# VISION-SJTU/UniDefense

Measured on AMD Instinct MI355X. Metric: images/sec fwd+bwd (256x256, EffNet-b4), higher is better.
Workload: dtype f32

## Files before the change

unidefense_amd/csrc/conv_mfma.hip:

```cpp
#include "pw_common.h"

namespace {

typedef _Float16 f16x2 __attribute__((ext_vector_type(2)));
typedef _Float16 f16x8 __attribute__((ext_vector_type(8)));
typedef uint32_t u32x2 __attribute__((ext_vector_type(2)));


constexpr int odd_slots(int bytes) { return (bytes / 16) % 2 == 0 ? bytes + 16 : bytes; }
constexpr int round_up(int v, int m) { return (v + m - 1) / m * m; }

template <int CIN_, int COUT_, int MODE_, int TH_, int TW_, int CK_, int TS_, int NW_ = 4>
struct Cfg {
    static constexpr int CIN = CIN_, COUT = COUT_, MODE = MODE_, TH = TH_, TW = TW_, CK = CK_, TS = TS_, NW = NW_, NT = 64 * NW_;
    static constexpr int CINP = round_up(CIN, 8), COUTP = round_up(COUT, 16), NTL = COUTP / 16;
    static constexpr int PIX = TH * TW, MW = PIX / 16 / NW;
    static constexpr int PH = MODE == 0 ? TH + 2 : MODE == 1 ? TH / 2 + 1 : 2 * TH + 1;
    static constexpr int PW = MODE == 0 ? TW + 2 : MODE == 1 ? TW / 2 + 1 : 2 * TW + 1;
    static constexpr int PROW = odd_slots(CINP * 2), PPLANE = PH * PW * PROW;
    static constexpr int NCC = CIN / CK, NSTAGE = (9 / TS) * NCC;
    static constexpr int CPT = round_up(CK, 8) / 8, NCH = TS * CPT;
    static constexpr int KSTEPS = (NCH + 3) / 4, KSP = KSTEPS * 32;
    static constexpr int WROW = odd_slots(KSP * 2), WPLANE = COUTP * WROW;
    static constexpr int LDS = 2 * PPLANE + 2 * WPLANE;
// ... 94 lines not shown
    int ty[MW], tx[MW];
#pragma unroll
    for (int mi = 0; mi < MW; ++mi) {
        const int p = (wave + NW * mi) * 16 + pl;
        if (MODE == 1) {
            constexpr int PC = C::PIX / 4, HW = TW / 2;
            const int cls = p / PC, r = p - cls * PC;
            ty[mi] = 2 * (r / HW) + (cls >> 1);
            tx[mi] = 2 * (r % HW) + (cls & 1);
        } else {
            ty[mi] = p / TW;
            tx[mi] = p % TW;
        }
    }

    f32x4 acc[MW][NTL];
#pragma unroll
    for (int mi = 0; mi < MW; ++mi)
#pragma unroll
        for (int nt = 0; nt < NTL; ++nt) acc[mi][nt] = f32x4{0.f, 0.f, 0.f, 0.f};

    int swe = 0, smin = 0;
    bool have = false;
#pragma unroll 1
    for (int stage = 0; stage < C::NSTAGE; ++stage) {
        const int tap0 = (stage / C::NCC) * TS, c0 = (stage % C::NCC) * CK;
        float mw = 0.f;
#pragma unroll
        for (int j = 0; j < NWI; ++j) mw = absmax4(mw, wr[j]);
        mw = ud_wave_max(mw);
        if (lane == 0) sred[stage & 1][wave] = mw;
        __syncthreads();
        mw = sred[stage & 1][0];
#pragma unroll
        for (int w = 1; w < NW; ++w) mw = fmaxf(mw, sred[stage & 1][w]);
        int ratio_e = 0;
        {
            const uint32_t bits = __float_as_uint(mw);
            const int ef = (int)(bits >> 23) & 0xff;
            if (ef != 0) {
                int want = 14 - (ef - 127);
                want = want < -100 ? -100 : want > 100 ? 100 : want;
                if (!have) {
                    swe = smin = want;
                    have = true;
                } else {
                    const int top = ef - 127 + swe;
                    if (top > 14 || top < 4) {
                        const int ne = want < smin + 80 ? want : smin + 80;
                        ratio_e = ne - swe;
                        swe = ne;
                        smin = ne < smin ? ne : smin;
                    }
                }
            }
        }
        const float sw = pow2f(swe);
#pragma unroll
        for (int j = 0; j < NWI; ++j) {
            const int i = t + j * NT;
            const int co = i / WQ, c4 = i - co * WQ;
            if (i < WITEMS) store_split4h(ws + co * WROW + c4 * 8, WPLANE, wr[j], sw);
        }
        if (stage + 1 < C::NSTAGE) wload(stage + 1);
        __syncthreads();
        if (ratio_e != 0) {
            const float ratio = pow2f(ratio_e < -126 ? -126 : ratio_e);
#pragma unroll
            for (int mi = 0; mi < MW; ++mi)
#pragma unroll
                for (int nt = 0; nt < NTL; ++nt) acc[mi][nt] *= ratio;
        }
        bool act[MW];
        bool any = false;
#pragma unroll
        for (int mi = 0; mi < MW; ++mi) {
            act[mi] = true;
            if (MODE == 1) {
                const int cls = (wave + NW * mi) / (C::PIX / 64);
                const int kh = tap0 / 3, kw = tap0 - 3 * kh;
                act[mi] = ((kh & 1) != (cls >> 1)) && ((kw & 1) != (cls & 1));
            }
            any = any || act[mi];
        }
        if (!any) continue;
#pragma unroll
        for (int ks = 0; ks < KSTEPS; ++ks) {
            const int q = ks * 4 + grp;
            f16x8 wf[NTL][2];
#pragma unroll
            for (int nt = 0; nt < NTL; ++nt) {
                const char* s = ws + (nt * 16 + pl) * WROW + q * 16;
                wf[nt][0] = *reinterpret_cast<const f16x8*>(s);
                wf[nt][1] = *reinterpret_cast<const f16x8*>(s + WPLANE);
            }
            const int qc = q < NCH ? q : NCH - 1;
            const int tl = qc / CPT, c8 = qc - tl * CPT;
            const int tap = tap0 + tl, kh = tap / 3, kw = tap - 3 * kh;
            const int coff = (c0 + c8 * 8) * 2;
#pragma unroll
            for (int mi = 0; mi < MW; ++mi) {
                if (!act[mi]) continue;
                int py, px;
                if (MODE == 0) {
                    py = ty[mi] + kh;
                    px = tx[mi] + kw;
                } else if (MODE == 1) {
                    py = (ty[mi] + 1 - kh) >> 1;
                    px = (tx[mi] + 1 - kw) >> 1;
                } else {
                    py = 2 * ty[mi] + kh;
                    px = 2 * tx[mi] + kw;
                }
                const char* s = patch + (py * PW + px) * PROW + coff;
                const f16x8 xh = *reinterpret_cast<const f16x8*>(s);
                const f16x8 xl = *reinterpret_cast<const f16x8*>(s + PPLANE);
#pragma unroll
                for (int nt = 0; nt < NTL; ++nt) {
                    f32x4 c = acc[mi][nt];
                    c = __builtin_amdgcn_mfma_f32_16x16x32_f16(wf[nt][1], xh, c, 0, 0, 0);
                    c = __builtin_amdgcn_mfma_f32_16x16x32_f16(wf[nt][0], xl, c, 0, 0, 0);
                    c = __builtin_amdgcn_mfma_f32_16x16x32_f16(wf[nt][0], xh, c, 0, 0, 0);
                    acc[mi][nt] = c;
                }
            }
        }
    }

    const float inv_sw = pow2f(-swe);
#pragma unroll
    for (int mi = 0; mi < MW; ++mi) {
        const int oh = oh0 + ty[mi], ow = ow0 + tx[mi];
        if (oh >= g.Hout || ow >= g.Wout) continue;
        float* dst = y + (((long)n * g.Hout + oh) * g.Wout + ow) * COUT;
#pragma unroll
        for (int nt = 0; nt < NTL; ++nt) {
            const int co = nt * 16 + grp * 4;
            if (co < COUT) *reinterpret_cast<f32x4*>(dst + co) = acc[mi][nt] * inv_sw * inv_sx;
        }
    }
}

template <class C>
int launch(const ud_conv_geom& g, const float* x, const float* wmat, float* y, hipStream_t s) {
    const int tiles_x = ud_cdiv(g.Wout, C::TW), tiles_y = ud_cdiv(g.Hout, C::TH);
    const long blocks = (long)g.N * tiles_x * tiles_y;
    if (blocks > 0x7fffffffL) return UD_EINVAL;
    hipLaunchKernelGGL((conv_mfma<C>), dim3((unsigned)blocks), dim3(C::NT), 0, s, g, x, wmat, y, tiles_x, tiles_y);
    UD_LAUNCH_CHECK();
    return 0;
}


template <int CIN_, int MA_, int MODE_, int CC_>
struct WCfg {
    static constexpr int CIN = CIN_, MA = MA_, MODE = MODE_, CC = CC_, S = MODE == 0 ? 1 : 2;
    static constexpr int PH = 3 * S + 3, PWP = 7 * S + 3;
    static constexpr int MAP = round_up(MA, 16), MT = MAP / 16, NY = CIN / CC;
    static constexpr int NC = 9 * CC, NTILES = round_up(NC, 16) / 16, NTW = (NTILES + 3) / 4;
    static constexpr int AROW = 80, APLANE = MAP * AROW;
    static constexpr int XPLANE = 3 * CC * PH * 16;
    static constexpr int LDS = 3 * APLANE + 3 * XPLANE;
    static_assert(MODE == 0 || MODE == 2, "gathers of a plain conv: stride 1 or 2, pad 1");
    static_assert(CIN % CC == 0 && CC % 4 == 0 && MA % 4 == 0, "16-byte runs");
    static_assert(LDS <= 65536, "two workgroups per CU");
};

__device__ __forceinline__ void store_split4t(char* dst, int plane, int stride, const f32x4& v) {
    uint32_t p[2][3];
    pw::split2(v[0], v[1], p[0][0], p[0][1], p[0][2]);
    pw::split2(v[2], v[3], p[1][0], p[1][1], p[1][2]);
#pragma unroll
    for (int c = 0; c < 4; ++c)
#pragma unroll
        for (int k = 0; k < 3; ++k) {
            const uint32_t w = p[c >> 1][k];
            *reinterpret_cast<uint16_t*>(dst + c * stride + k * plane) = (uint16_t)((c & 1) ? (w >> 16) : (w & 0xffffu));
        }
}

template <class C>
__global__ __launch_bounds__(256) void conv_mfma_wgrad(ud_conv_geom g, const float* __restrict__ a, const float* __restrict__ x,
                                                       float* __restrict__ part, int tiles_x, int tiles_y, int ntiles) {
    constexpr int CIN = C::CIN, MA = C::MA, CC = C::CC, S = C::S, PH = C::PH, PWP = C::PWP, MT = C::MT, NTW = C::NTW;
    constexpr int AROW = C::AROW, APLANE = C::APLANE, XPLANE = C::XPLANE, NC = C::NC, K = 9 * CIN;
    __shared__ __attribute__((aligned(16))) char sm[C::LDS];
    char* const at = sm;
    char* const xs = sm + 3 * APLANE;
    const int t = threadIdx.x, wave = t >> 6, lane = t & 63, pl = lane & 15, grp = lane >> 4;
    const int c0 = blockIdx.y * CC;
    f32x4 acc[MT][NTW];
#pragma unroll
    for (int mt = 0; mt < MT; ++mt)
#pragma unroll
        for (int j = 0; j < NTW; ++j) acc[mt][j] = f32x4{0.f, 0.f, 0.f, 0.f};
    int xoff[NTW];
#pragma unroll
    for (int j = 0; j < NTW; ++j) {
        int c = (wave + 4 * j) * 16 + pl;
        c = c < NC ? c : NC - 1;
        const int tap = c / CC, ci = c - tap * CC, kh = tap / 3, kw = tap - 3 * kh;
        xoff[j] = ((kw * CC + ci) * PH + S * grp + kh) * 16;
    }
    for (int tile = blockIdx.x; tile < ntiles; tile += gridDim.x) {
        int b = tile;
        const int tile_x = b % tiles_x;
        b /= tiles_x;
        const int tile_y = b % tiles_y, n = b / tiles_y;
        const int oh0 = tile_y * 4, ow0 = tile_x * 8, ih0 = S * oh0 - 1, iw0 = S * ow0 - 1;
        __syncthreads();
        {
            constexpr int Q = C::MAP / 4, ITEMS = 32 * Q;
            for (int i = t; i < ITEMS; i += 256) {
                const int p = i / Q, c4 = i - p * Q;
                const int oh = oh0 + (p >> 3), ow = ow0 + (p & 7);
                f32x4 v = {0.f, 0.f, 0.f, 0.f};
                if (c4 * 4 < MA && oh < g.Hout && ow < g.Wout)
                    v = *reinterpret_cast<const f32x4*>(a + (((long)n * g.Hout + oh) * g.Wout + ow) * MA + c4 * 4);
                store_split4t(at + c4 * 4 * AROW + p * 2, APLANE, AROW, v);
            }
        }
        {
            constexpr int Q = CC / 4, ITEMS = PH * PWP * Q;
            for (int i = t; i < ITEMS; i += 256) {
                const int pix = i / Q, c4 = i - pix * Q;
                const int py = pix / PWP, px = pix - py * PWP;
                const int ih = ih0 + py, iw = iw0 + px;
                f32x4 v = {0.f, 0.f, 0.f, 0.f};
                if (ih >= 0 && ih < g.Hin && iw >= 0 && iw < g.Win)
                    v = *reinterpret_cast<const f32x4*>(x + (((long)n * g.Hin + ih) * g.Win + iw) * CIN + c0 + c4 * 4);
#pragma unroll
                for (int kw = 0; kw < 3; ++kw) {
                    const int d = px - kw;
                    if (d >= 0 && d % S == 0 && d / S < 8)
                        store_split4t(xs + ((kw * CC + c4 * 4) * PH + py) * 16 + (d / S) * 2, XPLANE, PH * 16, v);
                }
            }
        }
        __syncthreads();
        pw::Frag3 af[MT];
#pragma unroll
        for (int mt = 0; mt < MT; ++mt) {
            const char* sp = at + (mt * 16 + pl) * AROW + grp * 16;
#pragma unroll
            for (int k = 0; k < 3; ++k) af[mt].p[k] = *reinterpret_cast<const pw::bf16x8*>(sp + k * APLANE);
        }
#pragma unroll
        for (int j = 0; j < NTW; ++j) {
            if ((wave + 4 * j) * 16 >= NC) continue;
            pw::Frag3 bf;
#pragma unroll
            for (int k = 0; k < 3; ++k) bf.p[k] = *reinterpret_cast<const pw::bf16x8*>(xs + xoff[j] + k * XPLANE);
#pragma unroll
            for (int mt = 0; mt < MT; ++mt) acc[mt][j] = pw::mma6(af[mt], bf, acc[mt][j]);
        }
    }
    float* dst = part + (long)blockIdx.x * MA * K;
#pragma unroll
    for (int j = 0; j < NTW; ++j) {
        const int c = (wave + 4 * j) * 16 + pl;
        if (c >= NC) continue;
        const int tap = c / CC, ci = c - tap * CC;
#pragma unroll
        for (int mt = 0; mt < MT; ++mt)
#pragma unroll
            for (int r = 0; r < 4; ++r) {
                const int ma = mt * 16 + grp * 4 + r;
                if (ma < MA) dst[(long)ma * K + tap * CIN + c0 + ci] = acc[mt][j][r];
            }
    }
}

int wgrad_parts(long ntiles, int Cin, int Ma, int ny) {
    long cap = 6L * 1024 * 1024 / ((long)Ma * 9 * Cin);
    if (cap > 512 / ny) cap = 512 / ny;
    long p = ntiles / 4;
    if (p > cap) p = cap;
    return p < 1 ? 1 : (int)p;
}

template <class C>
int launch_wgrad(const ud_conv_geom& g, const float* a, const float* x, float* part, float* out, hipStream_t s) {
    const int tiles_x = ud_cdiv(g.Wout, 8), tiles_y = ud_cdiv(g.Hout, 4);
    const long ntiles = (long)g.N * tiles_x * tiles_y;
    if (ntiles > 0x7fffffffL) return UD_EINVAL;
    const int parts = wgrad_parts(ntiles, C::CIN, C::MA, C::NY);
    hipLaunchKernelGGL((conv_mfma_wgrad<C>), dim3((unsigned)parts, (unsigned)C::NY), dim3(256), 0, s, g, a, x, part, tiles_x, tiles_y,
                       (int)ntiles);
    UD_LAUNCH_CHECK();
    return pw::fold_launch(part, parts, C::MA * 9 * C::CIN, out, nullptr, nullptr, 0, nullptr, nullptr, s);
}

int mode_of(const ud_conv_geom& g) {
    if (g.KH != 3 || g.KW != 3 || g.pad_t != 1 || g.pad_l != 1) return -1;
    if (!g.transposed && g.stride == 1 && g.Hout == g.Hin && g.Wout == g.Win) return 0;
    if (g.transposed && g.stride == 2 && g.Hout == 2 * g.Hin && g.Wout == 2 * g.Win) return 1;
    if (!g.transposed && g.stride == 2 && g.Hin == 2 * g.Hout && g.Win == 2 * g.Wout) return 2;
    return -1;
}

}

#define UD_CONV_MFMA_CASES(X)                                                                   \
    X(20, 20, 0, 16, 16, 20, 9, 4)                                                  \
    X(40, 20, 0, 8, 16, 40, 3, 4)                                                   \
    X(40, 40, 0, 8, 16, 40, 3, 4)                                                   \
    X(20, 40, 0, 8, 16, 20, 9, 4)                                                   \
    X(80, 40, 0, 8, 8, 80, 1, 4)                                                    \
    X(80, 80, 0, 8, 8, 40, 1, 4)                                                    \
    X(40, 80, 0, 8, 8, 40, 3, 4)                                                    \
    X(160, 80, 0, 4, 8, 40, 1, 2)    \
    X(80, 160, 0, 4, 8, 16, 1, 2)                                    \
    X(20, 20, 1, 16, 16, 20, 1, 4)                                                  \
    X(40, 40, 1, 16, 16, 40, 1, 4)                                                  \
    X(80, 80, 1, 8, 16, 80, 1, 4)                                                   \
    X(20, 20, 2, 8, 8, 20, 9, 4)                                                    \
    X(40, 40, 2, 8, 8, 40, 1, 4)                                                    \
    X(80, 80, 2, 4, 4, 40, 1, 1)

extern "C" {

int ud_conv_mfma_mode(const ud_conv_geom* g) { return g ? mode_of(*g) : -1; }

int ud_conv_mfma_supported(int Cin, int Cout, int mode) {
#define X(ci, co, m, th, tw, ck, ts, nw) \
    if (Cin == ci && Cout == co && mode == m) return 1;
    UD_CONV_MFMA_CASES(X)
#undef X
    return 0;
}

int ud_conv_mfma(const ud_conv_geom* g, const float* x, const float* wmat, float* y, int Cout, ud_stream_t stream) {
    if (!g || !x || !wmat || !y) return UD_EINVAL;
    const int mode = mode_of(*g);
    if (mode < 0 || !ud_conv_mfma_supported(g->Cin, Cout, mode)) return UD_EINVAL;
    if ((((uintptr_t)x | (uintptr_t)wmat | (uintptr_t)y) & 15) != 0) return UD_EINVAL;
    if (g->N < 1 || g->Hout < 1 || g->Wout < 1) return 0;
    hipStream_t s = (hipStream_t)stream;
#define X(ci, co, m, th, tw, ck, ts, nw) \
    if (g->Cin == ci && Cout == co && mode == m) return launch<Cfg<ci, co, m, th, tw, ck, ts, nw>>(*g, x, wmat, y, s);
    UD_CONV_MFMA_CASES(X)
#undef X
    return UD_EINVAL;
}

#define UD_CONV_MFMA_WGRAD_CASES(X) \
    X(160, 80, 0, 40) X(80, 80, 0, 40) X(80, 40, 0, 40) X(40, 40, 0, 40) X(40, 20, 0, 40) X(20, 20, 0, 20) \
    X(80, 80, 2, 20) X(40, 40, 2, 20) X(20, 20, 2, 20)

int ud_conv_mfma_wgrad_supported(int Cin, int Ma, int mode) {
#define X(ci, ma, m, cc) \
    if (Cin == ci && Ma == ma && mode == m) return 1;
    UD_CONV_MFMA_WGRAD_CASES(X)
#undef X
    return 0;
}

long ud_conv_mfma_wgrad_ws_floats(int Cin, int Ma) {
    if (Cin < 1 || Ma < 1) return UD_EINVAL;
    return (long)wgrad_parts(1L << 40, Cin, Ma, 1) * Ma * 9 * Cin;
}

int ud_conv_mfma_wgrad(const ud_conv_geom* g, const float* a, const float* x, float* part, float* out, int Ma, ud_stream_t stream) {
    if (!g || !a || !x || !part || !out) return UD_EINVAL;
    const int mode = mode_of(*g);
    if (mode < 0 || !ud_conv_mfma_wgrad_supported(g->Cin, Ma, mode)) return UD_EINVAL;
    if ((((uintptr_t)a | (uintptr_t)x) & 15) != 0) return UD_EINVAL;
    if (g->N < 1 || g->Hout < 1 || g->Wout < 1) return UD_EINVAL;
    hipStream_t s = (hipStream_t)stream;
#define X(ci, ma, m, cc) \
    if (g->Cin == ci && Ma == ma && mode == m) return launch_wgrad<WCfg<ci, ma, m, cc>>(*g, a, x, part, out, s);
    UD_CONV_MFMA_WGRAD_CASES(X)
#undef X
    return UD_EINVAL;
}

}
```

unidefense_amd/kernels.py:

```python
import ctypes as C
import math
import os

import torch

from . import lib as _lib
from .config import cfg as CFG
from .devmem import Scratch, ZeroPool
from .lib import ConvGeom, GemmDesc, GemmP3Desc

_call = _lib.call

GEMM_PROFILE = None


def _stream():
    return C.c_void_p(torch.cuda.current_stream().cuda_stream)


def _p(t):
    if t is None:
        return None
    return C.c_void_p(t.data_ptr())

# ... 948 lines not shown
        return gemm_nn(dy2, ctx.w, out=out, accumulate=out is not None)
    return _p2_run("nn", ctx.plans["nn"], _spectral_dy(ctx, dy2, dy_absmax), ctx.w, ctx.M, ctx.K, ctx.N, dy2, out=out)


def spectral_wgrad(ctx, dy2, dy_absmax=None):
    if ctx.plans is None:
        return gemm_tn(dy2, ctx.x)
    return _p2_run("tn", ctx.plans["tn"], _spectral_dy(ctx, dy2, dy_absmax), ctx.x, ctx.N, ctx.K, ctx.M, dy2)


def _p2_tune(key, x2, w2, M, N, Kd, forced, want_stats=False):
    dy2 = torch.randn(M, N, device=x2.device)
    acc = torch.zeros(2 * N, dtype=torch.float64, device=x2.device) if want_stats else None

    def fwd_x3():
        r = gemm_nt(x2, w2, stats=acc)
        if want_stats and not r[1]:
            colstats(r[0], acc)
    t_x3 = _time_launches(lambda: (fwd_x3(), gemm_nn(dy2, w2), gemm_tn(dy2, x2)))
    xp, wp, dp = split_planes(x2, prec=2), split_planes(w2, prec=2), split_planes(dy2, prec=2)
    t_p2 = _time_launches(lambda: (split_planes(x2, xp), split_planes(dy2, dp), split_planes(w2, wp)))
    t_stats = _time_launches(lambda: colstats(dy2, acc)) if want_stats else 0.0
    plans = []
    for kind, (a, b, m, n, k) in (("nt", (xp, wp, M, N, Kd)), ("nn", (dp, wp, M, Kd, N)), ("tn", (dp, xp, N, Kd, M))):
        best, best_t = None, 1e30
        for plan in _p2_plans(kind, m, n, k):
            st = acc if (kind == "nt" and want_stats) else None
            t = _time_launches(lambda: _p2_run(kind, plan, a, b, m, n, k, x2, stats=st))
            if st is not None and plan[0] != "plain":
                t += t_stats
            if t < best_t:
                best, best_t = plan, t
        plans.append(list(best))
        t_p2 += best_t
    res = plans if (forced or t_p2 < 0.97 * t_x3) else None
    _TUNED[key] = res
    _tune_cache_save()
    return res


_WG_SPLIT_MAXT = 512
_WG_SPLIT_TARGET = 768
_WG_SPLIT_ROWS = 256


def _pick_split(tiles, K):
    if tiles >= _WG_SPLIT_MAXT or K < 512:
        return 1
    s = min(max(1, K // _WG_SPLIT_ROWS), -(-_WG_SPLIT_TARGET // tiles))
    return max(1, min(s, 1024))


_TILE_CFGS = ((128, 128, 1.00), (128, 64, 0.93), (256, 32, 1.10), (32, 256, 1.10), (64, 128, 0.93))


_FWD_SPLIT_T = 224
_FWD_SPLIT_K = 512
_FWD_SPLIT_MINK = 256
_FWD_SPLIT_WGS = 320


def _fwd_split(M, N, K):
    t = _tiles(M, N)
    if t >= _FWD_SPLIT_T or K < _FWD_SPLIT_K:
        return 1
    return max(1, min(K // _FWD_SPLIT_MINK, -(-_FWD_SPLIT_WGS // t)))


_X3_MINDIM = 16


def _tiles(M, N):
    best, best_tiles = None, 1
    for bm, bn, pen in _TILE_CFGS:
        t = -(-M // bm) * -(-N // bn)
        cost = -(-t // 256) * bm * bn * pen
        if best is None or cost < best:
            best, best_tiles = cost, t
    return best_tiles


def gemm_tn(a, b):
    _act(a, b)
    K, M = a.shape
    N = b.shape[1]
    assert b.shape[0] == K
    split = _pick_split(_tiles(M, N), K)
    r = _tuned_launch("tn", a, b, None, M, N, K, M, N, 1, 1, False, None,
                      lambda scr: _gemm(a, b, scr, M, N, K, M, N, N, 1, 1, 2 if split > 1 else 0, split))
    if r is not None:
        return r
    if split > 1:
        out = split_out((M, N), a)
        return _gemm(a, b, out, M, N, K, M, N, N, 1, 1, 2, split)
    out = empty((M, N), a)
    return _gemm(a, b, out, M, N, K, M, N, N, 1, 1, 0, 1)


def conv_geom(N, Hin, Win, Cin, Hout, Wout, KH, KW, stride, pad_t, pad_l, transposed=0):
    g = ConvGeom()
    g.N, g.Hin, g.Win, g.Cin, g.Hout, g.Wout = N, Hin, Win, Cin, Hout, Wout
    g.KH, g.KW, g.stride, g.pad_t, g.pad_l, g.transposed = KH, KW, stride, pad_t, pad_l, transposed
    return g


_CONV_SPLITK = True


_CONV_SMALL = True
_CONV_SMALL_MIN_M = 262144
_CONV_SMALL_OK = {}


def _conv_small_supported(Ci, Co, KH, KW):
    key = (Ci, Co, KH, KW)
    if key not in _CONV_SMALL_OK:
        _CONV_SMALL_OK[key] = _call("ud_conv_small_supported", Ci, Co, KH, KW) == 1
    return _CONV_SMALL_OK[key]


_CONV_SMALL_WS = Scratch(torch.float32)
_CONV_SMALL_WGRAD_OK = {}


def _conv_small_wgrad_supported(Ci, Ma, KH, KW):
    key = (Ci, Ma, KH, KW)
    if key not in _CONV_SMALL_WGRAD_OK:
        _CONV_SMALL_WGRAD_OK[key] = _call("ud_conv_small_wgrad_supported", Ci, Ma, KH, KW) == 1
    return _CONV_SMALL_WGRAD_OK[key]


_CONV_MFMA = True
_CONV_MFMA_MIN_M = 16384
_CONV_MFMA_SHAPES = frozenset({(20, 20, 0), (40, 20, 0), (40, 40, 0), (20, 40, 0), (80, 40, 0), (80, 80, 0), (40, 80, 0),
                               (20, 20, 1), (40, 40, 1), (80, 80, 1), (20, 20, 2)})
_CONV_MFMA_OK = {}


def _conv_mfma_mode(g):
    return int(_lib.load().ud_conv_mfma_mode(C.byref(g)))


def _conv_mfma_takes(g, Co, M, *tensors):
    if not _CONV_MFMA or M < _CONV_MFMA_MIN_M:
        return False
    key = (g.Cin, Co, _conv_mfma_mode(g))
    if key[2] < 0 or (_CONV_MFMA_SHAPES is not None and key not in _CONV_MFMA_SHAPES):
        return False
    if key not in _CONV_MFMA_OK:
        _CONV_MFMA_OK[key] = _call("ud_conv_mfma_supported", *key) == 1
    return _CONV_MFMA_OK[key] and all(t.dtype == torch.float32 and t.data_ptr() % 16 == 0 for t in tensors)


_CONV_MFMA_WGRAD_SHAPES = frozenset()
_CONV_MFMA_WGRAD_OK = {}
_CONV_MFMA_WS = Scratch(torch.float32)


def _conv_mfma_wgrad_takes(g, Ma, M, *tensors):
    if not _CONV_MFMA or M < _CONV_MFMA_MIN_M:
        return False
    key = (g.Cin, Ma, _conv_mfma_mode(g))
    if key[2] not in (0, 2) or (_CONV_MFMA_WGRAD_SHAPES is not None and key not in _CONV_MFMA_WGRAD_SHAPES):
        return False
    if key not in _CONV_MFMA_WGRAD_OK:
        _CONV_MFMA_WGRAD_OK[key] = _call("ud_conv_mfma_wgrad_supported", *key) == 1
    return _CONV_MFMA_WGRAD_OK[key] and all(t.dtype == torch.float32 and t.data_ptr() % 16 == 0 for t in tensors)


def conv_gather_nt(x, wmat, g):
    _chk(x, wmat)
    M = g.N * g.Hout * g.Wout
    K = g.KH * g.KW * g.Cin
    Co = wmat.shape[0]
    assert wmat.shape[1] == K and x.numel() == g.N * g.Hin * g.Win * g.Cin
    if _conv_mfma_takes(g, Co, M, x, wmat):
        out = empty((g.N, g.Hout, g.Wout, Co), x)
        _call("ud_conv_mfma", C.byref(g), _p(x), _p(wmat), _p(out), Co, _stream())
        return out
    if _CONV_SMALL and M >= _CONV_SMALL_MIN_M and _conv_small_supported(g.Cin, Co, g.KH, g.KW):
        out = empty((g.N, g.Hout, g.Wout, Co), x)
        _call("ud_conv_small", C.byref(g), _p(x), _p(wmat), _p(out), Co, _stream())
        return out
    split = _fwd_split(M, Co, K) if _CONV_SPLITK else 1
    if g.Cin % 4 == 0:
        gk = (g.Hin, g.Win, g.Cin, g.KH, g.KW, g.stride, g.transposed)
        tmp = []

        def scratch():
            if not tmp:
                tmp.append(empty((M, Co), x))
            return tmp[0]
        tuned = _tuned_plan(("conv",) + gk, M, Co, K,
                            lambda cfg, sp: _gemm(x, wmat, scratch(), M, Co, K, 0, K, Co, 2, 0, 2 if sp > 1 else 0, sp, geom=g, cfg=cfg),
                            lambda: _gemm(x, wmat, scratch(), M, Co, K, 0, K, Co, 2, 0, 2 if split > 1 else 0, split, geom=g))
        if tuned is not None:
            cfg, sp = tuned
            out = (split_out if sp > 1 else empty)((g.N, g.Hout, g.Wout, Co), x)
            _gemm(x, wmat, out, M, Co, K, 0, K, Co, 2, 0, 2 if sp > 1 else 0, sp, geom=g, cfg=cfg)
            return out
    if split > 1:
        out = split_out((g.N, g.Hout, g.Wout, Co), x)
        _gemm(x, wmat, out, M, Co, K, 0, K, Co, 2, 0, 2, split, geom=g)
        return out
    out = empty((g.N, g.Hout, g.Wout, Co), x)
    _gemm(x, wmat, out, M, Co, K, 0, K, Co, 2, 0, geom=g)
    return out


_STEM_DGRAD_OK = {}


def stem_dgrad_supported(Ci, Co, KH, KW, stride):
    key = (Ci, Co, KH, KW, stride)
    if key not in _STEM_DGRAD_OK:
        _STEM_DGRAD_OK[key] = _call("ud_stem_dgrad_supported", Ci, Co, KH, KW, stride) == 1
    return _STEM_DGRAD_OK[key]


def stem_dgrad(dy, w, g, out=None):
    Co = w.shape[0]
    if not stem_dgrad_supported(g.Cin, Co, g.KH, g.KW, g.stride):
        raise ValueError(f"no stem data-gradient kernel for Cin {g.Cin}, Cout {Co}, {g.KH}x{g.KW} / {g.stride}")
    dy = dy.contiguous()
    w = w.contiguous()
    _chk(dy, w, out)
    assert dy.numel() == g.N * g.Hout * g.Wout * Co and w.numel() == Co * 3 * g.KH * g.KW and dy.data_ptr() % 16 == 0
    acc = out is not None
    if acc:
        assert out.is_contiguous() and out.dtype == torch.float32 and out.numel() == g.N * 3 * g.Hin * g.Win
    else:
        out = empty((g.N, 3, g.Hin, g.Win), dy)
    _call("ud_stem_dgrad", C.byref(g), _p(dy), _p(w), _p(out), Co, 1 if acc else 0, _stream())
    return out


def absdiff_bwd(a, b, g):
    _chk(a, b, g)
    db = torch.empty_like(b)
    _call("ud_absdiff_bwd", _p(a), _p(b), _p(g), None, _p(db), b.numel(), _stream())
    return db


def outer(u, v):
    _chk(u, v)
    M, D = u.numel(), v.numel()
    out = empty((M, D), u)
    _call("ud_outer", _p(u), _p(v), _p(out), M, D, _stream())
    return out


def _chk_same(*ts):
    _chk(*ts)
    if any(t.shape != ts[0].shape for t in ts):
        raise ValueError(f"shapes differ: {[tuple(t.shape) for t in ts]}")


def _chk_f64(t, n):
    if not (t.is_cuda and t.dtype == torch.float64 and t.is_contiguous() and t.numel() >= n):
        raise ValueError(f"expected a contiguous float64 CUDA tensor of at least {n} values, got {t.dtype} {t.device} "
                         f"shape={tuple(t.shape)}")


def attack_step_linf(x_adv, x0, g, step, eps, lo, hi):
    _chk_same(x_adv, x0, g)
    _call("ud_attack_step_linf", _p(x_adv), _p(x0), _p(g), x_adv.numel(), float(step), float(eps), float(lo), float(hi),
          _stream())
    return x_adv


def sample_sumsq_ws_bytes(N, per):
    return _call("ud_sample_sumsq_ws_bytes", int(N), int(per))


def sample_sumsq(a, b=None, out=None, ws=None):
    _chk_same(*((a,) if b is None else (a, b)))
    N = a.shape[0]
    per = a.numel() // N
    need = sample_sumsq_ws_bytes(N, per)
    if out is None:
        out = torch.empty(N, dtype=torch.float64, device=a.device)
    _chk_f64(out, N)
    if ws is None and need:
        ws = torch.empty(need // 8, dtype=torch.float64, device=a.device)
    if need:
        _chk_f64(ws, need // 8)
    _call("ud_sample_sumsq", _p(a), _p(b), N, per, _p(out), _p(ws) if need else None, ws.numel() * 8 if need else 0, _stream())
    return out


def attack_step_l2(x_adv, g, gss, step):
    _chk_same(x_adv, g)
    N = x_adv.shape[0]
    _chk_f64(gss, N)
    _call("ud_attack_step_l2", _p(x_adv), _p(g), _p(gss), N, x_adv.numel() // N, float(step), _stream())
    return x_adv


def attack_project_l2(x_adv, x0, dss, eps, lo, hi):
    _chk_same(x_adv, x0)
    N = x_adv.shape[0]
    _chk_f64(dss, N)
    _call("ud_attack_project_l2", _p(x_adv), _p(x0), _p(dss), N, x_adv.numel() // N, float(eps), float(lo), float(hi),
          _stream())
    return x_adv


# ... 1850 lines not shown
```

Measured before the change: 1367.

## Rewrite MFMA weight-gradient conv with double-buffered f16 split and enable shapes

The weight-gradient 3x3 conv kernel is restructured. Tiles are now prefetched into registers and stored into a double-buffered LDS stage while the previous tile computes. The bf16 three-way split with six MFMAs is replaced by a scaled f16 hi/lo split using three 16x16x32 f16 MFMAs and transposed LDS reads, with running exponent tracking that rescales accumulators. It also makes tile sizes configurable and enables the kernel for most shapes in the Python dispatch, which was previously empty. The risks are numerical accuracy of the dynamic f16 scaling and extra per-tile reductions and syncs.

```diff
diff --git a/unidefense_amd/csrc/conv_mfma.hip b/unidefense_amd/csrc/conv_mfma.hip
--- a/unidefense_amd/csrc/conv_mfma.hip
+++ b/unidefense_amd/csrc/conv_mfma.hip
@@ -270,43 +270,68 @@
 }
 
 
-template <int CIN_, int MA_, int MODE_, int CC_>
+template <int CIN_, int MA_, int MODE_, int CC_, int TH_, int TW_>
 struct WCfg {
-    static constexpr int CIN = CIN_, MA = MA_, MODE = MODE_, CC = CC_, S = MODE == 0 ? 1 : 2;
-    static constexpr int PH = 3 * S + 3, PWP = 7 * S + 3;
+    static constexpr int CIN = CIN_, MA = MA_, MODE = MODE_, CC = CC_, TH = TH_, TW = TW_, S = MODE == 0 ? 1 : 2;
+    static constexpr int PIX = TH * TW, KS = PIX / 32;
+    static constexpr int PH = S * (TH - 1) + 3, PW = S * (TW - 1) + 3, PPIX = PH * PW;
     static constexpr int MAP = round_up(MA, 16), MT = MAP / 16, NY = CIN / CC;
-    static constexpr int NC = 9 * CC, NTILES = round_up(NC, 16) / 16, NTW = (NTILES + 3) / 4;
-    static constexpr int AROW = 80, APLANE = MAP * AROW;
-    static constexpr int XPLANE = 3 * CC * PH * 16;
-    static constexpr int LDS = 3 * APLANE + 3 * XPLANE;
+    static constexpr int NC = 9 * CC, NB = round_up(NC, 16) / 16, NTW = (NB + 3) / 4;
+    static constexpr int AROW = odd_slots(MAP * 2), APLANE = PIX * AROW;
+    static constexpr int PROW = (CC * 2) % 16 == 8 ? CC * 2 : odd_slots(CC * 2), XPLANE = PPIX * PROW;
+    static constexpr int STAGE = round_up(2 * (APLANE + XPLANE), 16), LDS = 2 * STAGE;
+    static constexpr int QA = MA / 4, AITEMS = PIX * QA, NIA = (AITEMS + 255) / 256;
+    static constexpr int QX = CC / 4, XITEMS = PPIX * QX, NIX = (XITEMS + 255) / 256;
     static_assert(MODE == 0 || MODE == 2, "gathers of a plain conv: stride 1 or 2, pad 1");
-    static_assert(CIN % CC == 0 && CC % 4 == 0 && MA % 4 == 0, "16-byte runs");
-    static_assert(LDS <= 65536, "two workgroups per CU");
+    static_assert(CIN % CC == 0 && CC % 4 == 0 && MA % 4 == 0, "16-byte runs; a 4-column set of the result has one tap");
+    static_assert(TW % 8 == 0 && PIX % 32 == 0, "a lane group's 8 pixels lie in one tile row");
+    static_assert(NIA <= 32 && NIX <= 32, "validity masks");
+    static_assert(LDS + 64 <= 65536, "two workgroups per CU");
 };
 
-__device__ __forceinline__ void store_split4t(char* dst, int plane, int stride, const f32x4& v) {
-    uint32_t p[2][3];
-    pw::split2(v[0], v[1], p[0][0], p[0][1], p[0][2]);
-    pw::split2(v[2], v[3], p[1][0], p[1][1], p[1][2]);
-#pragma unroll
-    for (int c = 0; c < 4; ++c)
-#pragma unroll
-        for (int k = 0; k < 3; ++k) {
-            const uint32_t w = p[c >> 1][k];
-            *reinterpret_cast<uint16_t*>(dst + c * stride + k * plane) = (uint16_t)((c & 1) ? (w >> 16) : (w & 0xffffu));
-        }
+struct Frag2 { f16x8 hi, lo; };
+__device__ __forceinline__ Frag2 read_cols2(const pw::lds_char* s, int plane, int row_stride) {
+    typedef __attribute__((address_space(3))) pw::s16x4 lds_s16x4;
+    const pw::s16x4 h0 = __builtin_amdgcn_ds_read_tr16_b64_v4i16((lds_s16x4*)(s));
+    const pw::s16x4 h1 = __builtin_amdgcn_ds_read_tr16_b64_v4i16((lds_s16x4*)(s + 4 * row_stride));
+    const pw::s16x4 l0 = __builtin_amdgcn_ds_read_tr16_b64_v4i16((lds_s16x4*)(s + plane));
+    const pw::s16x4 l1 = __builtin_amdgcn_ds_read_tr16_b64_v4i16((lds_s16x4*)(s + plane + 4 * row_stride));
+    Frag2 f;
+    f.hi = __builtin_bit_cast(f16x8, __builtin_shufflevector(h0, h1, 0, 1, 2, 3, 4, 5, 6, 7));
+    f.lo = __builtin_bit_cast(f16x8, __builtin_shufflevector(l0, l1, 0, 1, 2, 3, 4, 5, 6, 7));
+    return f;
+}
+__device__ __forceinline__ f32x4 mma3(const Frag2& a, const Frag2& b, f32x4 c) {
+    c = __builtin_amdgcn_mfma_f32_16x16x32_f16(a.lo, b.hi, c, 0, 0, 0);
+    c = __builtin_amdgcn_mfma_f32_16x16x32_f16(a.hi, b.lo, c, 0, 0, 0);
+    c = __builtin_amdgcn_mfma_f32_16x16x32_f16(a.hi, b.hi, c, 0, 0, 0);
+    return c;
+}
+__device__ __forceinline__ void follow_max(uint32_t bits, int& e, bool& have) {
+    const int ef = (int)(bits >> 23) & 0xff;
+    if (ef == 0) return;
+    int want = 14 - (ef - 127);
+    want = want < -100 ? -100 : want > 100 ? 100 : want;
+    const int top = ef - 127 + e;
+    if (!have || top > 14 || top < 8) e = want;
+    have = true;
 }
 
 template <class C>
-__global__ __launch_bounds__(256) void conv_mfma_wgrad(ud_conv_geom g, const float* __restrict__ a, const float* __restrict__ x,
-                                                       float* __restrict__ part, int tiles_x, int tiles_y, int ntiles) {
-    constexpr int CIN = C::CIN, MA = C::MA, CC = C::CC, S = C::S, PH = C::PH, PWP = C::PWP, MT = C::MT, NTW = C::NTW;
-    constexpr int AROW = C::AROW, APLANE = C::APLANE, XPLANE = C::XPLANE, NC = C::NC, K = 9 * CIN;
+__global__ __launch_bounds__(256, 2) void conv_mfma_wgrad(ud_conv_geom g, const float* __restrict__ a, const float* __restrict__ x,
+                                                          float* __restrict__ part, int tiles_x, int tiles_y, int ntiles) {
+    constexpr int CIN = C::CIN, MA = C::MA, CC = C::CC, S = C::S, TH = C::TH, TW = C::TW, PW = C::PW, MT = C::MT, NTW = C::NTW;
+    constexpr int AROW = C::AROW, APLANE = C::APLANE, PROW = C::PROW, XPLANE = C::XPLANE, NC = C::NC, K = 9 * CIN;
+    constexpr int QA = C::QA, QX = C::QX, NIA = C::NIA, NIX = C::NIX;
     __shared__ __attribute__((aligned(16))) char sm[C::LDS];
-    char* const at = sm;
-    char* const xs = sm + 3 * APLANE;
-    const int t = threadIdx.x, wave = t >> 6, lane = t & 63, pl = lane & 15, grp = lane >> 4;
+    __shared__ float sred[4][2];
+    const pw::lds_char* const smr = (const pw::lds_char*)sm;
+    const int t = threadIdx.x, lane = t & 63, pl = lane & 15, grp = lane >> 4, q = pl >> 2, pp = pl & 3;
+    const int wave = __builtin_amdgcn_readfirstlane(t >> 6);
     const int c0 = blockIdx.y * CC;
+
+    for (int i = t; i < C::LDS / 16; i += 256) reinterpret_cast<pw::u32x4*>(sm)[i] = pw::u32x4{0u, 0u, 0u, 0u};
+
     f32x4 acc[MT][NTW];
 #pragma unroll
     for (int mt = 0; mt < MT; ++mt)
@@ -315,64 +340,158 @@
     int xoff[NTW];
 #pragma unroll
     for (int j = 0; j < NTW; ++j) {
-        int c = (wave + 4 * j) * 16 + pl;
-        c = c < NC ? c : NC - 1;
+        int c = ((wave + 4 * j) * 4 + pp) * 4;
+        c = c < NC ? c : NC - 4;
         const int tap = c / CC, ci = c - tap * CC, kh = tap / 3, kw = tap - 3 * kh;
-        xoff[j] = ((kw * CC + ci) * PH + S * grp + kh) * 16;
-    }
-    for (int tile = blockIdx.x; tile < ntiles; tile += gridDim.x) {
+        xoff[j] = (kh * PW + kw + S * q) * PROW + ci * 2;
+    }
+
+    f32x4 ra[NIA], rx[NIX];
+    uint32_t va = 0u, vx = 0u;
+    auto load = [&](int tile) __attribute__((always_inline)) {
         int b = tile;
         const int tile_x = b % tiles_x;
         b /= tiles_x;
         const int tile_y = b % tiles_y, n = b / tiles_y;
-        const int oh0 = tile_y * 4, ow0 = tile_x * 8, ih0 = S * oh0 - 1, iw0 = S * ow0 - 1;
-        __syncthreads();
-        {
-            constexpr int Q = C::MAP / 4, ITEMS = 32 * Q;
-            for (int i = t; i < ITEMS; i += 256) {
-                const int p = i / Q, c4 = i - p * Q;
-                const int oh = oh0 + (p >> 3), ow = ow0 + (p & 7);
-                f32x4 v = {0.f, 0.f, 0.f, 0.f};
-                if (c4 * 4 < MA && oh < g.Hout && ow < g.Wout)
-                    v = *reinterpret_cast<const f32x4*>(a + (((long)n * g.Hout + oh) * g.Wout + ow) * MA + c4 * 4);
-                store_split4t(at + c4 * 4 * AROW + p * 2, APLANE, AROW, v);
-            }
-        }
-        {
-            constexpr int Q = CC / 4, ITEMS = PH * PWP * Q;
-            for (int i = t; i < ITEMS; i += 256) {
-                const int pix = i / Q, c4 = i - pix * Q;
-                const int py = pix / PWP, px = pix - py * PWP;
-                const int ih = ih0 + py, iw = iw0 + px;
-                f32x4 v = {0.f, 0.f, 0.f, 0.f};
-                if (ih >= 0 && ih < g.Hin && iw >= 0 && iw < g.Win)
-                    v = *reinterpret_cast<const f32x4*>(x + (((long)n * g.Hin + ih) * g.Win + iw) * CIN + c0 + c4 * 4);
-#pragma unroll
-                for (int kw = 0; kw < 3; ++kw) {
-                    const int d = px - kw;
-                    if (d >= 0 && d % S == 0 && d / S < 8)
-                        store_split4t(xs + ((kw * CC + c4 * 4) * PH + py) * 16 + (d / S) * 2, XPLANE, PH * 16, v);
+        const int oh0 = tile_y * TH, ow0 = tile_x * TW, ih0 = S * oh0 - 1, iw0 = S * ow0 - 1;
+        va = vx = 0u;
+#pragma unroll
+        for (int j = 0; j < NIA; ++j) {
+            const int i = t + j * 256;
+            const int p = i / QA, c4 = i - p * QA;
+            const int oh = oh0 + p / TW, ow = ow0 + p % TW;
+            const bool ok = i < C::AITEMS && oh < g.Hout && ow < g.Wout;
+            const long off = (((long)n * g.Hout + min(oh, g.Hout - 1)) * g.Wout + min(ow, g.Wout - 1)) * MA + c4 * 4;
+            ra[j] = *reinterpret_cast<const f32x4*>(a + off);
+            va |= ok ? 1u << j : 0u;
+        }
+#pragma unroll
+        for (int j = 0; j < NIX; ++j) {
+            const int i = t + j * 256;
+            const int pix = i / QX, c4 = i - pix * QX;
+            const int py = pix / PW, px = pix - py * PW;
+            const int ih = ih0 + py, iw = iw0 + px;
+            const bool ok = i < C::XITEMS && ih >= 0 && ih < g.Hin && iw >= 0 && iw < g.Win;
+            const long off = (((long)n * g.Hin + min(max(ih, 0), g.Hin - 1)) * g.Win + min(max(iw, 0), g.Win - 1)) * CIN + c0 + c4 * 4;
+            rx[j] = *reinterpret_cast<const f32x4*>(x + off);
+            vx |= ok ? 1u << j : 0u;
+        }
+    };
+    auto maxima = [&]() __attribute__((always_inline)) {
+        const f32x4 zero = {0.f, 0.f, 0.f, 0.f};
+        float m0 = 0.f, m1 = 0.f;
+#pragma unroll
+        for (int j = 0; j < NIA; ++j) {
+            ra[j] = (va >> j) & 1u ? ra[j] : zero;
+            m0 = absmax4(m0, ra[j]);
+        }
+#pragma unroll
+        for (int j = 0; j < NIX; ++j) {
+            rx[j] = (vx >> j) & 1u ? rx[j] : zero;
+            m1 = absmax4(m1, rx[j]);
+        }
+        m0 = ud_wave_max(m0);
+        m1 = ud_wave_max(m1);
+        if (lane == 0) {
+            sred[wave][0] = m0;
+            sred[wave][1] = m1;
+        }
+    };
+    int ea = 0, ex = 0, emin = 0;
+    bool have_a = false, have_x = false, have = false;
+    auto store = [&](int buf) __attribute__((always_inline)) {
+        const float m0 = fmaxf(fmaxf(sred[0][0], sred[1][0]), fmaxf(sred[2][0], sred[3][0]));
+        const float m1 = fmaxf(fmaxf(sred[0][1], sred[1][1]), fmaxf(sred[2][1], sred[3][1]));
+        const int e_old = ea + ex;
+        follow_max(__float_as_uint(m0), ea, have_a);
+        follow_max(__float_as_uint(m1), ex, have_x);
+        const bool live = have_a && have_x;
+        if (live && have && ea + ex > emin + 80) ea = emin + 80 - ex;
+        const int e_new = ea + ex;
+        if (e_new != e_old) {
+            int r = e_new - e_old;
+            r = r < -126 ? -126 : r > 127 ? 127 : r;
+            const float ratio = pow2f(r);
+#pragma unroll
+            for (int mt = 0; mt < MT; ++mt)
+#pragma unroll
+                for (int j = 0; j < NTW; ++j) acc[mt][j] *= ratio;
+        }
+        if (live) {
+            emin = !have || e_new < emin ? e_new : emin;
+            have = true;
+        }
+        const float sx = pow2f(ex);
+        char* const ab = sm + buf * C::STAGE;
+        char* const xb = ab + 2 * APLANE;
+#pragma unroll
+        for (int j = 0; j < NIA; ++j) {
+            const int i = t + j * 256;
+            const int p = i / QA, c4 = i - p * QA;
+            const int e1 = ea < -100 ? -100 : ea;
+            if (i < C::AITEMS) store_split4h(ab + p * AROW + c4 * 8, APLANE, ra[j] * pow2f(ea - e1 < -126 ? -126 : ea - e1), pow2f(e1));
+        }
+#pragma unroll
+        for (int j = 0; j < NIX; ++j) {
+            const int i = t + j * 256;
+            const int pix = i / QX, c4 = i - pix * QX;
+            if (i < C::XITEMS) store_split4h(xb + pix * PROW + c4 * 8, XPLANE, rx[j], sx);
+        }
+    };
+    auto compute = [&](int buf) __attribute__((always_inline)) {
+        const pw::lds_char* const ab = smr + buf * C::STAGE + (8 * grp + q) * AROW + pp * 8;
+        const pw::lds_char* const xb = smr + buf * C::STAGE + 2 * APLANE;
+#pragma unroll
+        for (int ks = 0; ks < C::KS; ++ks) {
+            const int p = 32 * ks + 8 * grp;
+            const pw::lds_char* const xk = xb + (S * (p / TW) * PW + S * (p % TW)) * PROW;
+            if constexpr (MT <= 3) {
+                Frag2 af[MT];
+#pragma unroll
+                for (int mt = 0; mt < MT; ++mt) af[mt] = read_cols2(ab + ks * 32 * AROW + mt * 32, APLANE, AROW);
+#pragma unroll
+                for (int j = 0; j < NTW; ++j) {
+                    if ((3 + 4 * j) * 16 >= NC && (wave + 4 * j) * 16 >= NC) continue;
+                    const Frag2 bf = read_cols2(xk + xoff[j], XPLANE, S * PROW);
+#pragma unroll
+                    for (int mt = 0; mt < MT; ++mt) acc[mt][j] = mma3(af[mt], bf, acc[mt][j]);
+                }
+            } else {
+#pragma unroll
+                for (int mt = 0; mt < MT; ++mt) {
+                    asm volatile("" ::: "memory");
+                    const Frag2 af = read_cols2(ab + ks * 32 * AROW + mt * 32, APLANE, AROW);
+#pragma unroll
+                    for (int j = 0; j < NTW; ++j) {
+                        if ((3 + 4 * j) * 16 >= NC && (wave + 4 * j) * 16 >= NC) continue;
+                        const Frag2 bf = read_cols2(xk + xoff[j], XPLANE, S * PROW);
+                        acc[mt][j] = mma3(af, bf, acc[mt][j]);
+                    }
                 }
             }
         }
+    };
+
+    const int gx = gridDim.x, last = ntiles - 1;
+    int tile = blockIdx.x;
+    load(tile);
+    maxima();
+    __syncthreads();
+    store(0);
+    load(min(tile + gx, last));
+    __syncthreads();
+    for (int it = 0;; ++it) {
+        compute(it & 1);
+        tile += gx;
+        if (tile >= ntiles) break;
+        maxima();
         __syncthreads();
-        pw::Frag3 af[MT];
-#pragma unroll
-        for (int mt = 0; mt < MT; ++mt) {
-            const char* sp = at + (mt * 16 + pl) * AROW + grp * 16;
-#pragma unroll
-            for (int k = 0; k < 3; ++k) af[mt].p[k] = *reinterpret_cast<const pw::bf16x8*>(sp + k * APLANE);
-        }
-#pragma unroll
-        for (int j = 0; j < NTW; ++j) {
-            if ((wave + 4 * j) * 16 >= NC) continue;
-            pw::Frag3 bf;
-#pragma unroll
-            for (int k = 0; k < 3; ++k) bf.p[k] = *reinterpret_cast<const pw::bf16x8*>(xs + xoff[j] + k * XPLANE);
-#pragma unroll
-            for (int mt = 0; mt < MT; ++mt) acc[mt][j] = pw::mma6(af[mt], bf, acc[mt][j]);
-        }
-    }
+        store((it & 1) ^ 1);
+        load(min(tile + gx, last));
+        __syncthreads();
+    }
+    const int e1 = ea < -100 ? -100 : ea, e2 = ea - e1 < -126 ? -126 : ea - e1;
+    const float ia1 = pow2f(-e1), ia2 = pow2f(-e2 > 127 ? 127 : -e2), ix = pow2f(-ex);
     float* dst = part + (long)blockIdx.x * MA * K;
 #pragma unroll
     for (int j = 0; j < NTW; ++j) {
@@ -384,7 +503,7 @@
 #pragma unroll
             for (int r = 0; r < 4; ++r) {
                 const int ma = mt * 16 + grp * 4 + r;
-                if (ma < MA) dst[(long)ma * K + tap * CIN + c0 + ci] = acc[mt][j][r];
+                if (ma < MA) dst[(long)ma * K + tap * CIN + c0 + ci] = acc[mt][j][r] * ix * ia1 * ia2;
             }
     }
 }
@@ -399,9 +518,9 @@
 
 template <class C>
 int launch_wgrad(const ud_conv_geom& g, const float* a, const float* x, float* part, float* out, hipStream_t s) {
-    const int tiles_x = ud_cdiv(g.Wout, 8), tiles_y = ud_cdiv(g.Hout, 4);
+    const int tiles_x = ud_cdiv(g.Wout, C::TW), tiles_y = ud_cdiv(g.Hout, C::TH);
     const long ntiles = (long)g.N * tiles_x * tiles_y;
-    if (ntiles > 0x7fffffffL) return UD_EINVAL;
+    if (ntiles > 0x3fffffffL) return UD_EINVAL;
     const int parts = wgrad_parts(ntiles, C::CIN, C::MA, C::NY);
     hipLaunchKernelGGL((conv_mfma_wgrad<C>), dim3((unsigned)parts, (unsigned)C::NY), dim3(256), 0, s, g, a, x, part, tiles_x, tiles_y,
                        (int)ntiles);
@@ -463,11 +582,12 @@
 }
 
 #define UD_CONV_MFMA_WGRAD_CASES(X) \
-    X(160, 80, 0, 40) X(80, 80, 0, 40) X(80, 40, 0, 40) X(40, 40, 0, 40) X(40, 20, 0, 40) X(20, 20, 0, 20) \
-    X(80, 80, 2, 20) X(40, 40, 2, 20) X(20, 20, 2, 20)
+    X(160, 80, 0, 20, 4, 8)  X(80, 80, 0, 20, 4, 8)  X(80, 40, 0, 40, 4, 8)  \
+    X(40, 40, 0, 40, 4, 8)   X(40, 20, 0, 40, 4, 8)  X(20, 20, 0, 20, 8, 8)  \
+    X(80, 80, 2, 20, 4, 8)   X(40, 40, 2, 20, 4, 8)  X(20, 20, 2, 20, 4, 8)
 
 int ud_conv_mfma_wgrad_supported(int Cin, int Ma, int mode) {
-#define X(ci, ma, m, cc) \
+#define X(ci, ma, m, cc, th, tw) \
     if (Cin == ci && Ma == ma && mode == m) return 1;
     UD_CONV_MFMA_WGRAD_CASES(X)
 #undef X
@@ -486,8 +606,8 @@
     if ((((uintptr_t)a | (uintptr_t)x) & 15) != 0) return UD_EINVAL;
     if (g->N < 1 || g->Hout < 1 || g->Wout < 1) return UD_EINVAL;
     hipStream_t s = (hipStream_t)stream;
-#define X(ci, ma, m, cc) \
-    if (g->Cin == ci && Ma == ma && mode == m) return launch_wgrad<WCfg<ci, ma, m, cc>>(*g, a, x, part, out, s);
+#define X(ci, ma, m, cc, th, tw) \
+    if (g->Cin == ci && Ma == ma && mode == m) return launch_wgrad<WCfg<ci, ma, m, cc, th, tw>>(*g, a, x, part, out, s);
     UD_CONV_MFMA_WGRAD_CASES(X)
 #undef X
     return UD_EINVAL;
diff --git a/unidefense_amd/kernels.py b/unidefense_amd/kernels.py
--- a/unidefense_amd/kernels.py
+++ b/unidefense_amd/kernels.py
@@ -1124,7 +1124,7 @@
     return _CONV_MFMA_OK[key] and all(t.dtype == torch.float32 and t.data_ptr() % 16 == 0 for t in tensors)
 
 
-_CONV_MFMA_WGRAD_SHAPES = frozenset()
+_CONV_MFMA_WGRAD_SHAPES = frozenset({(80, 80, 0), (80, 40, 0), (40, 40, 0), (40, 20, 0), (20, 20, 0), (40, 40, 2), (20, 20, 2)})
 _CONV_MFMA_WGRAD_OK = {}
 _CONV_MFMA_WS = Scratch(torch.float32)
 
```

Measured after the change: 1376, median of 6. About the same (+0.7%).
